# neeek2303/EMOPortraits

Measured on AMD Instinct MI355X. Metric: reenactment frames/sec @512x512, 1-src->N-driver, higher is better.
Workload: dtype f32

## Files before the change

### emoportraits_amd/csrc/conv_inst_f16x2_up2.hip

```cpp
#include "conv_dispatch.h"
#include "conv_igemm_bf16x3.h"
#include "conv_split_pair_common.h"

#ifndef EMO_UP2_CHAIN
#define EMO_UP2_CHAIN 1
#endif
#ifndef EMO_UP2_LOADS_EARLY
#define EMO_UP2_LOADS_EARLY 1
#endif

struct ConvCfgUp2 {
  static constexpr int BM = 64, TM = 2, TP = 2, KC = 16, NPL = 2;
  static constexpr int TRL = 2, TWL = 64;
  static constexpr int PR = TRL + 2, NQ = TWL / 4, NQ1 = NQ + 1;
  static constexpr int SUB = ((PR * NQ1 + 4 + 11) / 16) * 16 + 4;
  static constexpr int CHS = 4 * SUB, NG = 2, QPG = 128, NHQ = 2 * PR;
  static constexpr int WPLANE = 2 * BM;
  static constexpr int WTAP = NPL * WPLANE;
  static constexpr int WST = 8 * WTAP;
  static constexpr int WST_BYTES = WST * 16;
  static constexpr int PPL = NG * CHS, PBUF = NPL * PPL;
  static constexpr int SCT = 1024;
  static constexpr int OFF_P = 0, OFF_W = 2 * PBUF, OFF_SCT = OFF_W + WST;
  static constexpr int WSTRIDE = WST + (2 * SCT + BM) / 4;
  static constexpr int OFF_BIAS_F = OFF_SCT * 4 + 2 * SCT;
  static constexpr int EPI_CS = 4 * 132 + 4;
  static constexpr int OFF_IMG_F = (OFF_W + WSTRIDE) * 4;
  static constexpr int LDS_BYTES = (OFF_IMG_F + 32 * EPI_CS) * 4;
  static_assert(OFF_IMG_F >= OFF_BIAS_F + BM, "the epilogue image spares the patch buffers, W[0], the tables and the bias: a chained successor's");
  static_assert(32 * EPI_CS * 4 >= WST_BYTES, "W[1] lies inside the image's allocation");
  static_assert(WST_BYTES == 32 * 1024, "eight 1 KiB pieces per wave and half-stage");
  static_assert(PR * NQ + NHQ <= QPG, "one interior quad or one halo pixel per thread and stage");
  static_assert(LDS_BYTES <= 160 * 1024, "LDS");
};

__global__ __launch_bounds__(256) __attribute__((amdgpu_waves_per_eu(1, 1)))
void conv_igemm_f16x2_up2_kernel(const ConvArgs a) {
  using Cfg = ConvCfgUp2;
  using opx8 = halfx8;
  constexpr int NPL = 2, NPROD = 3;
  constexpr int BM = Cfg::BM, TM = Cfg::TM, TP = Cfg::TP, KC = Cfg::KC;
  constexpr int PR = Cfg::PR, NQ = Cfg::NQ, NQ1 = Cfg::NQ1, SUB = Cfg::SUB, CHS = Cfg::CHS, QPG = Cfg::QPG;
  constexpr int NHQ = Cfg::NHQ, PPL = Cfg::PPL, PBUF = Cfg::PBUF;
  constexpr bool UPS = false;
  constexpr int TW = Cfg::TWL, TWS = Cfg::TWL;

  extern __shared__ __attribute__((aligned(16))) float smem[];

  const int tid = threadIdx.x;
  const int lane = tid & 63;
  const int wave = __builtin_amdgcn_readfirstlane(tid >> 6);
  const int half = lane >> 5, l32 = lane & 31;
  const int wq = wave & 1;
  const int p0 = (wave >> 1) * TP * 32;
  float sat_m = 0.0f;

  const int HW = a.H * a.W;
  const bool has_affine = a.scale != nullptr;
  const float in_scale = a.in_scale;
  constexpr float CLAMP_HI = 65504.0f;
  const float clamp_lo = a.relu_in ? 0.0f : -CLAMP_HI;
  const int nst = a.n_cchunks;
  const int nptiles = a.tiles_x * a.tiles_y;

  const int q_u = tid % QPG;
  const int q_g = __builtin_amdgcn_readfirstlane(tid / QPG);
  const bool is_quad = q_u < PR * NQ;
  const int hq = q_u - PR * NQ;
  const bool is_halo = !is_quad && hq < NHQ;
  const int h_side = hq & 1;
  const int q_r = is_quad ? q_u / NQ : (is_halo ? hq >> 1 : 0);
  const int q_c = is_quad ? q_u - q_r * NQ : 0;
  int q_slb[4];
#pragma unroll
  for (int i = 0; i < 4; ++i) {
    const int dump = q_g * CHS + i * SUB + PR * NQ1 + (q_u & 3);
    const int own = is_quad ? q_g * CHS + i * SUB + q_r * NQ1 + q_c : q_g * CHS + h_side * SUB + q_r * NQ1 + NQ;
    q_slb[i] = ((is_quad || (is_halo && i == (h_side ? 0 : 3))) ? own : dump) * 16;
  }

  floatx16 acc_lo[2][TM][TP], acc_hi[2][TM][TP];

  const int q8 = a.n_work >> 3, r8 = a.n_work & 7;
  const int xcd = blockIdx.x & 7;
  const int n_mine = q8 + (xcd < r8 ? 1 : 0);
  const int l_base = xcd < r8 ? xcd * (q8 + 1) : r8 * (q8 + 1) + (xcd - r8) * q8;
  const int l_stride = (gridDim.x + 7) >> 3;
#define EMO_U_WPTR(c_, k_, p_) (reinterpret_cast<const char*>(a.wpk) + ((long)((c_) * nst + (k_)) * 2 + (p_)) * Cfg::WST_BYTES)

  const int a_off = (half * BM + l32) * 16;
  EMO_P_DECLARE_B_OFF()

  const char* const lds_c = reinterpret_cast<const char*>(smem);
  char* const lds_w = reinterpret_cast<char*>(smem);
  opx8 fa_[2][NPL][TM], fb_[2][NPL][TP];
#define EMO_U_LOAD_FRAGS_PLANE(set_, pl_, hb_, pbyte_, a_, b_)                                        \
  {                                                                                                   \
    _Pragma("unroll") for (int i = 0; i < TM; ++i)                                                    \
      fa_[set_][pl_][i] = *reinterpret_cast<const opx8*>(lds_c + a_off + (Cfg::OFF_W + (hb_) * Cfg::WSTRIDE + \
          ((wq * 4 + (a_) * 2 + (b_)) * NPL + (pl_)) * Cfg::WPLANE + i * 32) * 16);                   \
    _Pragma("unroll") for (int j = 0; j < TP; ++j)                                                    \
      fb_[set_][pl_][j] = *reinterpret_cast<const opx8*>(lds_c + (EMO_P_B_OFF(j, (hb_) + (a_), wq + (b_)) + (pbyte_)) + ((pl_) * PPL) * 16); \
  }

  float* const sct = smem + Cfg::OFF_SCT * 4;
  const unsigned smem_lds = (unsigned)(size_t)(__attribute__((address_space(3))) char*)reinterpret_cast<char*>(smem);
  const unsigned lane16 = (unsigned)lane * 16u;

  floatx4 qv[8];
  float q_lo, q_hi;
  int q_tix;
  floatx4 q_sc, q_sh;
  opx8 cv_h, cv_m;
  emo_intx4 xrs = emo_raw_buffer(a.x);
  unsigned usoff[8];
#pragma unroll
  for (int u = 0; u < 8; ++u) usoff[u] = (unsigned)__builtin_amdgcn_readfirstlane((int)((unsigned)u * (unsigned)HW * 4u));
  unsigned lq_off = 0;
  bool lq_ok = false;
  unsigned q_vo;
#define EMO_U_ISSUE_BEGIN(st_)                                                                        \
  {                                                                                                   \
    const int c0_ = (st_) * KC + q_g * 8;                                                             \
    const bool cv_ = c0_ < a.Cin;                                                                     \
    const int cs_ = cv_ ? c0_ : 0;                                                                    \
    const bool keep_ = lq_ok && cv_;                                                                  \
    q_lo = keep_ ? clamp_lo : 0.0f;                                                                   \
    q_hi = keep_ ? CLAMP_HI : 0.0f;                                                                   \
    q_vo = lq_off + (unsigned)cs_ * (unsigned)HW * 4u;                                                \
    q_tix = (has_affine ? cs_ : (cs_ & (Cfg::SCT - 1))) >> 2;                                         \
  }
#define EMO_U_ISSUE_LOADS(u0_, u1_)                                                                   \
  { _Pragma("unroll") for (int u = (u0_); u < (u1_); u += 2) emo_bload4x2_pinned(xrs, q_vo, usoff[u], usoff[u + 1], qv[u], qv[u + 1]); }
#define EMO_U_HALF_TABLE(hf_)                                                                         \
  {                                                                                                   \
    const floatx4* t4_ = reinterpret_cast<const floatx4*>(sct) + q_tix + (hf_);                       \
    q_sc = t4_[0]; q_sh = t4_[Cfg::SCT / 4];                                                          \
  }
#define EMO_U_TOUCH_QUAD() { _Pragma("unroll") for (int u = 0; u < 8; ++u) emo_touch4(qv[u]); }
#define EMO_U_CONV_PIXEL(pbyte_, i_)                                                                  \
  {                                                                                                   \
    _Pragma("unroll") for (int hf_ = 0; hf_ < 2; ++hf_) {                                             \
      EMO_U_HALF_TABLE(hf_)                                                                           \
      float t_[4];                                                                                    \
      _Pragma("unroll") for (int k = 0; k < 4; ++k)                                                   \
        t_[k] = __fmaf_rn(qv[4 * hf_ + k][i_], q_sc[k], q_sh[k]);                                     \
      sat_m = __builtin_fmaxf(__builtin_fmaxf(sat_m, __builtin_fabsf(t_[0])), __builtin_fabsf(t_[1])); \
      sat_m = __builtin_fmaxf(__builtin_fmaxf(sat_m, __builtin_fabsf(t_[2])), __builtin_fabsf(t_[3])); \
      _Pragma("unroll") for (int k = 0; k < 4; k += 2)                                                \
        emo_split_f16x2_pair(__builtin_amdgcn_fmed3f(t_[k], q_lo, q_hi), __builtin_amdgcn_fmed3f(t_[k + 1], q_lo, q_hi), \
                             cv_h, cv_m, 4 * hf_ + k);                                                \
    }                                                                                                 \
    char* d_ = lds_w + (q_slb[i_] + (pbyte_));                                                        \
    *reinterpret_cast<opx8*>(d_) = cv_h;                                                              \
    *reinterpret_cast<opx8*>(d_ + PPL * 16) = cv_m;                                                   \
  }
#define EMO_U_DMA_PIECE(ptr_, wb_, k_)                                                                \
  {                                                                                                   \
    const int j_ = wave + 4 * (k_);                                                                   \
    emo_dma16_pinned_s((ptr_) + j_ * 1024, lane16, smem_lds + (unsigned)((Cfg::OFF_W + (wb_) * Cfg::WSTRIDE) * 16 + j_ * 1024)); \
  }

  constexpr int PA3[3] = {1, 0, 0}, PB3[3] = {0, 1, 0};
  constexpr int NTE = Cfg::SCT / 256;

#define EMO_U_DECODE(P_, L_)                                                                          \
  {                                                                                                   \
    const int l_ = (L_);                                                                              \
    P_##cotile = __builtin_amdgcn_readfirstlane(l_ % a.n_cotiles);                                    \
    const int rest_ = l_ / a.n_cotiles;                                                               \
    P_##n = __builtin_amdgcn_readfirstlane(rest_ / nptiles);                                          \
    const int lt_ = rest_ - P_##n * nptiles;                                                          \
    P_##x0 = __builtin_amdgcn_readfirstlane((lt_ % a.tiles_x) * Cfg::TWL);        \
    P_##y0 = __builtin_amdgcn_readfirstlane((lt_ / a.tiles_x) * Cfg::TRL);                            \
  }
#define EMO_U_CURSOR_OF(P_, ok_, off_)                                                                \
  {                                                                                                   \
    const int q_y_ = P_##y0 - 1 + q_r;                                                                \
    const int q_x_ = is_quad ? P_##x0 + 4 * q_c : (h_side ? P_##x0 + TWS : P_##x0 - 4);               \
    ok_ = (is_quad || is_halo) && (unsigned)q_y_ < (unsigned)a.H && q_x_ >= 0 && q_x_ < a.W;          \
    off_ = ok_ ? (unsigned)(q_y_ * a.W + q_x_) * 4u : 0u;                                             \
  }
#define EMO_U_NEXT_STAGE_BEGIN()                                                                      \
  {                                                                                                   \
    const bool sw_ = chain_out && cg + 2 == nst;                                                      \
    const int tgt_ = (chain_out && cg + 2 >= nst) ? cg + 2 - nst : (cg + 2 < nst ? cg + 2 : nst - 1); \
    lq_ok = sw_ ? nxq_ok : lq_ok;                                                                     \
    lq_off = sw_ ? nxq_off : lq_off;                                                                  \
    EMO_U_ISSUE_BEGIN(tgt_)                                                                           \
  }
#if EMO_S_TIMING == 2
#define EMO_U_LOOP_BARRIER(n_)                                                                        \
  {                                                                                                   \
    const unsigned long long b0_ = __builtin_amdgcn_s_memtime();                                      \
    asm volatile("s_waitcnt vmcnt(%0) lgkmcnt(0)" ::"n"(n_) : "memory");                              \
    const unsigned long long b1_ = __builtin_amdgcn_s_memtime();                                      \
    asm volatile("s_waitcnt lgkmcnt(0)\n\ts_barrier" ::: "memory");                                  \
    const unsigned long long b2_ = __builtin_amdgcn_s_memtime();                                      \
    asm volatile("s_waitcnt lgkmcnt(0)" ::: "memory");                                                \
    tw_wait += b1_ - b0_; tw_bar += b2_ - b1_; ++tw_n;                                                \
  }
#else
#define EMO_U_LOOP_BARRIER(n_) EMO_P_BARRIER(n_)
#endif

  constexpr bool CHAIN = EMO_UP2_CHAIN != 0, LOADS_EARLY = EMO_UP2_LOADS_EARLY != 0;
  float te_b = 0.0f;
  bool chained_in = false;
  int pp = 0;
  for (int idx8 = blockIdx.x >> 3; idx8 < n_mine; idx8 += l_stride) {
#if EMO_S_TIMING
    unsigned long long tstamp[12];
    for (int k = 0; k < 12; ++k) tstamp[k] = 0;
    unsigned long long tw_wait = 0, tw_bar = 0, tw_n = 0;
#endif
    EMO_S_STAMP(0)
    int cotile, it_n, x0, y0;
    {
      int it_cotile, it_x0, it_y0;
      EMO_U_DECODE(it_, l_base + idx8)
      cotile = it_cotile; x0 = it_x0; y0 = it_y0;
    }
    int nx_cotile = 0, nx_n = 0, nx_x0 = 0, nx_y0 = 0;
    bool chain_out = false, nxq_ok = false;
    unsigned nxq_off = 0;
    if (CHAIN && idx8 + l_stride < n_mine) {
      EMO_U_DECODE(nx_, l_base + idx8 + l_stride)
      chain_out = nx_n == it_n && nst >= 2;
      EMO_U_CURSOR_OF(nx_, nxq_ok, nxq_off)
    }
    xrs = emo_raw_buffer(a.x + (long)it_n * a.Cin * HW);
    asm volatile("" : "=v"(cv_h));
    asm volatile("" : "=v"(cv_m));
    if (CHAIN && chained_in) {
      if (tid < BM) smem[Cfg::OFF_BIAS_F + tid] = te_b;
      const char* const w1_ = EMO_U_WPTR(cotile, 0, 1);
      EMO_U_DMA_PIECE(w1_, 1, 0)
      EMO_U_DMA_PIECE(w1_, 1, 1)
      EMO_P_BARRIER(40);
    } else {
      {
        int it_x0 = x0, it_y0 = y0;
        EMO_U_CURSOR_OF(it_, lq_ok, lq_off)
      }
#pragma unroll
      for (int u = 0; u < 8; ++u) asm volatile("" : "=v"(qv[u]));
      {
        const char* const w0_ = EMO_U_WPTR(cotile, 0, 0);
#pragma unroll
        for (int k = 0; k < 8; ++k) EMO_U_DMA_PIECE(w0_, 0, k)
        const char* const w1_ = EMO_U_WPTR(cotile, 0, 1);
        EMO_U_DMA_PIECE(w1_, 1, 0)
        EMO_U_DMA_PIECE(w1_, 1, 1)
      }
      EMO_U_ISSUE_BEGIN(0)
      EMO_U_ISSUE_LOADS(0, 8)
#pragma unroll
      for (int k = 0; k < NTE; ++k) {
        const int c = tid + 256 * k;
        if (c < min(a.Cin, Cfg::SCT)) {
          const bool real = has_affine;
          sct[c] = (real ? a.scale[(long)it_n * a.Cin + c] : 1.0f) * in_scale;
          sct[Cfg::SCT + c] = (real ? a.shift[(long)it_n * a.Cin + c] : 0.0f) * in_scale;
        }
      }
      if (tid < BM) smem[Cfg::OFF_BIAS_F + tid] = a.bias != nullptr ? a.bias[cotile * BM + tid] : 0.0f;
      EMO_P_WAIT(0);
      EMO_U_TOUCH_QUAD()
      __syncthreads();
#pragma unroll
      for (int i = 0; i < 4; ++i) EMO_U_CONV_PIXEL(Cfg::OFF_P * 16, i)
      EMO_U_ISSUE_BEGIN(nst > 1 ? 1 : 0)
      EMO_U_ISSUE_LOADS(0, 8)
      EMO_P_BARRIER(0);
      EMO_U_TOUCH_QUAD()
      pp = 0;
    }

    EMO_S_STAMP(1)
#pragma unroll
    for (int c = 0; c < 2; ++c)
#pragma unroll
      for (int i = 0; i < TM; ++i)
#pragma unroll
        for (int j = 0; j < TP; ++j)
#pragma unroll
          for (int r = 0; r < 16; ++r) { acc_lo[c][i][j][r] = 0.0f; acc_hi[c][i][j][r] = 0.0f; }
    {
      const int pb0_ = (Cfg::OFF_P + pp * PBUF) * 16;
#pragma unroll
      for (int pl = 0; pl < NPL; ++pl) EMO_U_LOAD_FRAGS_PLANE(0, pl, 0, pb0_, 0, 0)
    }
    for (int cg = 0; cg < nst; ++cg) {
      const int pcur_b = (Cfg::OFF_P + pp * PBUF) * 16, pnxt_b = (Cfg::OFF_P + (pp ^ 1) * PBUF) * 16;
      const bool last_ = cg + 1 >= nst;
#pragma unroll
      for (int h = 0; h < 2; ++h) {
        const bool past_ = last_ && chain_out;
        const bool have1_ = CHAIN || h == 0 || !last_, have2_ = !last_ || (CHAIN && h == 0);
        const int ce_ = past_ ? nx_cotile : cotile, ke_ = last_ ? (chain_out ? 0 : nst - 1) : cg + 1;
        const char* const dma1 = h == 0 ? EMO_U_WPTR(cotile, cg, 1) : EMO_U_WPTR(ce_, ke_, 0);
        const char* const dma2 = EMO_U_WPTR(ce_, ke_, h);
        if (EMO_CONV_SETPRIO) __builtin_amdgcn_s_setprio(1);
#pragma unroll
        for (int gs = 0; gs < 4; ++gs) {
          const int fcur = (h * 4 + gs) & 1, fnxt = fcur ^ 1;
          if (gs == 3) { EMO_U_LOOP_BARRIER(0); }
          if (gs == 3 && h == 1) EMO_U_TOUCH_QUAD()
          if (!LOADS_EARLY && gs == 0 && h == 1) EMO_U_NEXT_STAGE_BEGIN()
          __builtin_amdgcn_sched_barrier(0);
          {
            const int an = gs < 3 ? (gs + 1) >> 1 : 0, bn = gs < 3 ? (gs + 1) & 1 : 0;
            const int hbn = gs < 3 ? h : h ^ 1;
            const int pbn = (gs == 3 && h == 1) ? pnxt_b : pcur_b;
#pragma unroll
            for (int pl = 0; pl < NPL; ++pl) {
              EMO_U_LOAD_FRAGS_PLANE(fnxt, pl, hbn, pbn, an, bn)
              if (gs < 3 && have1_) EMO_U_DMA_PIECE(dma1, h ^ 1, 2 + 2 * gs + pl)
              if (gs == 3 && have2_) EMO_U_DMA_PIECE(dma2, h, pl)
              if (!LOADS_EARLY && h == 1 && gs == 0) EMO_U_ISSUE_LOADS(2 * pl, 2 * pl + 2)
              if (!LOADS_EARLY && h == 1 && gs > 0 && gs < 3 && pl == 0) EMO_U_ISSUE_LOADS(2 + 2 * gs, 4 + 2 * gs)
            }
          }
          if (h == 0) EMO_U_CONV_PIXEL(pnxt_b, gs)
          if (LOADS_EARLY && h == 0 && gs == 3) {
            EMO_U_NEXT_STAGE_BEGIN()
            EMO_U_ISSUE_LOADS(0, 8)
          }
#pragma unroll
          for (int p = 0; p < NPROD; ++p) {
            const int pa = PA3[p], pb = PB3[p];
#pragma unroll
            for (int i = 0; i < TM; ++i)
#pragma unroll
              for (int j = 0; j < TP; ++j) {
                floatx16& acc_ = (pa == 0 && pb == 0) ? acc_lo[h][i][j] : acc_hi[h][i][j];
                acc_ = __builtin_amdgcn_mfma_f32_32x32x16_f16(fb_[fcur][pb][j], fa_[fcur][pa][i], acc_, 0, 0, 0);
              }
          }
          __builtin_amdgcn_sched_barrier(0);
        }
        if (EMO_CONV_SETPRIO) __builtin_amdgcn_s_setprio(0);
      }
      pp ^= 1;
    }

    EMO_S_STAMP(2)
    EMO_P_WAIT(0);
    EMO_S_STAMP(5)
    __syncthreads();
    EMO_S_STAMP(6)
    EMO_S_STAMP(7)
    float* const img = smem + Cfg::OFF_IMG_F;
    if (CHAIN && chain_out && tid < BM) te_b = a.bias != nullptr ? a.bias[nx_cotile * BM + tid] : 0.0f;
    const bool want_stats = a.gn_stats != nullptr;
    const int Ho = a.Hl, Wo = a.Wl;
    const unsigned oplane = (unsigned)Ho * Wo;
    const int tiles_xo = Wo / 64;
    const int ec = tid >> 4, eu = tid & 15;
#pragma unroll
    for (int i = 0; i < TM; ++i) {
#pragma unroll
      for (int p = 0; p < 2; ++p)
#pragma unroll
        for (int j = 0; j < TP; ++j)
#pragma unroll
          for (int r = 0; r < 16; ++r) {
            const float v = (emo_acc_read(acc_lo[p][i][j][r]) + emo_acc_read(acc_hi[p][i][j][r])) * a.out_scale;
            const int m = (r >> 2) * 8 + half * 4 + (r & 3);
            const int hr = 2 * (wave >> 1) + p, col = 2 * (j * 32 + m) + wq;
            img[l32 * Cfg::EPI_CS + hr * 132 + col] = v;
          }
      __syncthreads();
#pragma unroll
      for (int cc = 0; cc < 2; ++cc) {
        const int c = cc * 16 + ec;
        const int co = cotile * BM + i * 32 + c;
        const float bs = smem[Cfg::OFF_BIAS_F + i * 32 + c];
        float* const obase = a.out + ((long)it_n * a.Cout + co) * oplane;
        float s_[2] = {0.0f, 0.0f};
        floatx4 v_[4][2];
#pragma unroll
        for (int hr = 0; hr < 4; ++hr)
#pragma unroll
          for (int k = 0; k < 2; ++k) {
            floatx4 v = *reinterpret_cast<const floatx4*>(img + c * Cfg::EPI_CS + hr * 132 + 4 * eu + 64 * k);
            v = v + floatx4{bs, bs, bs, bs};
            v_[hr][k] = v;
            float* const op = obase + (unsigned)(2 * y0 + hr) * Wo + (2 * x0 + 4 * eu + 64 * k);
            if (EMO_CONV_NT_STORE) __builtin_nontemporal_store(v, reinterpret_cast<floatx4*>(op));
            else *reinterpret_cast<floatx4*>(op) = v;
            s_[k] += (v[0] + v[1]) + (v[2] + v[3]);
          }
        if (want_stats) {
          emo_row16_sum_n<2>(s_);
          float m2_[2] = {0.0f, 0.0f};
#pragma unroll
          for (int k = 0; k < 2; ++k) {
            s_[k] *= 1.0f / 256.0f;
#pragma unroll
            for (int hr = 0; hr < 4; ++hr)
#pragma unroll
              for (int e = 0; e < 4; ++e) {
                const float d = v_[hr][k][e] - s_[k];
                m2_[k] = __fmaf_rn(d, d, m2_[k]);
              }
          }
          emo_row16_sum_n<2>(m2_);
          if (eu == 0) {
#pragma unroll
            for (int k = 0; k < 2; ++k) {
              const int ptile = (y0 >> 1) * tiles_xo + (x0 >> 5) + k;
              reinterpret_cast<float2*>(a.gn_stats)[((long)it_n * (oplane / 256) + ptile) * a.Cout + co] = make_float2(s_[k], m2_[k]);
            }
          }
        }
      }
      if (i == 0) {
        EMO_S_STAMP(8)
        __syncthreads();
      }
    }
    EMO_S_STAMP(9)
#if EMO_S_TIMING
    EMO_S_STAMP(3)
    asm volatile("s_waitcnt vmcnt(0)" ::: "memory");
    EMO_S_STAMP(4)
    {
      const int ep_L_ = l_base + idx8;
      if (tid == 0 && ep_L_ < EMO_S_TLOG_N) {
        unsigned long long* t_ = emo_s_tlog + (long)ep_L_ * EMO_S_TLOG_W;
#pragma unroll
        for (int k = 0; k < 12; ++k) t_[k] = tstamp[k];
        t_[12] = (unsigned long long)__builtin_amdgcn_s_getreg((31 << 11) | 4);
        t_[13] = (unsigned long long)__builtin_amdgcn_s_getreg((31 << 11) | 20);
        t_[14] = (unsigned long long)blockIdx.x;
        t_[15] = (unsigned long long)(chained_in ? 1 : 0);
      }
      if (EMO_S_TIMING == 2 && lane == 0 && ep_L_ < EMO_S_TLOG_N / 8) {
        unsigned long long* w_ = emo_s_tlog + ((long)EMO_S_TLOG_N / 4 + (long)ep_L_ * 4 + wave) * EMO_S_TLOG_W;
        w_[0] = tw_wait; w_[1] = tw_bar; w_[2] = tw_n; w_[3] = tstamp[2] - tstamp[1];
      }
    }
#endif
    __syncthreads();
    chained_in = chain_out;
  }
  if (a.sat_flag != nullptr && sat_m > 65504.0f) *a.sat_flag = 1;
#undef EMO_U_WPTR
#undef EMO_U_DECODE
#undef EMO_U_CURSOR_OF
#undef EMO_U_NEXT_STAGE_BEGIN
#undef EMO_U_LOOP_BARRIER
#undef EMO_U_LOAD_FRAGS_PLANE
#undef EMO_U_ISSUE_BEGIN
#undef EMO_U_ISSUE_LOADS
#undef EMO_U_HALF_TABLE
#undef EMO_U_TOUCH_QUAD
#undef EMO_U_CONV_PIXEL
#undef EMO_U_DMA_PIECE
}

int conv_f16x2_up2_launch(ConvArgs a, hipStream_t s) {
  using Cfg = ConvCfgUp2;
  if (a.KD != 1 || a.D != 1 || a.ksplit != 1 || a.res != nullptr || a.act != EMO_ACT_NONE || a.run_if != nullptr) return EMO_ERR_UNSUPPORTED;
  if (a.Cout % Cfg::BM || a.Cin % 8 || (a.scale && a.Cin > Cfg::SCT)) return EMO_ERR_UNSUPPORTED;
  if (a.W % Cfg::TWL || a.H % Cfg::TRL) return EMO_ERR_UNSUPPORTED;
  if ((reinterpret_cast<unsigned long long>(a.x) & 15ull) || (reinterpret_cast<unsigned long long>(a.out) & 15ull)) return EMO_ERR_ALIGN;
  if ((unsigned long long)a.Cin * a.H * a.W * 4ull >= (1ull << 32) || (long)a.Hl * a.Wl >= (1l << 31)) return EMO_ERR_UNSUPPORTED;
  const long nt = (long)(a.W / Cfg::TWL) * (a.H / Cfg::TRL);
  const int cot = a.Cout / Cfg::BM;
  if (a.N > 65535 || nt * cot * a.N > 0x7fffffffL) return EMO_ERR_UNSUPPORTED;
  auto kern = conv_igemm_f16x2_up2_kernel;
  const int rc = emo_raise_dynamic_lds(kern);
  if (rc != EMO_OK) return rc;
  a.tiles_x = a.W / Cfg::TWL;
  a.tiles_y = a.H / Cfg::TRL;
  a.tiles_z = 1;
  a.n_cchunks = (a.Cin + Cfg::KC - 1) / Cfg::KC;
  a.stages_per_split = a.n_cchunks;
  a.partial = nullptr;
  a.cot0 = 0;
  a.n_cotiles = cot;
  a.n_work = (int)(nt * cot * a.N);
  const int ncu = emo_cu_count();
  const int grid = a.n_work > ncu ? ncu : a.n_work;
  hipLaunchKernelGGL(kern, dim3((unsigned)grid), dim3(256), (size_t)Cfg::LDS_BYTES, s, a);
  return emo_launch_status();
}

#if EMO_S_TIMING
extern "C" int emo_debug_conv_timing_up2(unsigned long long* host_out, int n_items) {
  if (!host_out || n_items < 0 || n_items > EMO_S_TLOG_N) return EMO_ERR_BAD_ARG;
  if (hipDeviceSynchronize() != hipSuccess) return EMO_ERR_BAD_ARG;
  return hipMemcpyFromSymbol(host_out, HIP_SYMBOL(emo_s_tlog), (size_t)n_items * EMO_S_TLOG_W * sizeof(unsigned long long)) == hipSuccess ? EMO_OK : EMO_ERR_BAD_ARG;
}
#endif
```

Before: 401.0.

## Double up2 conv tile height and merge split accumulators into one set

Raises the low-res tile from 2 to 4 rows (TP 2→4) so each weight stage feeds twice as many pixels, cutting weight DMA per output. It drops the lo/hi split accumulators so register use stays bounded, and chains the MFMAs into a single accumulator. The epilogue becomes a row-pair-by-row-pair pass with a smaller LDS image and more barriers, and it adds a partial-tile guard for heights not divisible by 4. Risks are a longer serial MFMA dependency chain, more epilogue syncs and fewer work items for load balance.

Result: faster. 413.1, median of 6 (+3.0%).

```diff
diff --git a/emoportraits_amd/csrc/conv_inst_f16x2_up2.hip b/emoportraits_amd/csrc/conv_inst_f16x2_up2.hip
--- a/emoportraits_amd/csrc/conv_inst_f16x2_up2.hip
+++ b/emoportraits_amd/csrc/conv_inst_f16x2_up2.hip
@@ -10,8 +10,8 @@
 #endif
 
 struct ConvCfgUp2 {
-  static constexpr int BM = 64, TM = 2, TP = 2, KC = 16, NPL = 2;
-  static constexpr int TRL = 2, TWL = 64;
+  static constexpr int BM = 64, TM = 2, TP = 4, KC = 16, NPL = 2;
+  static constexpr int TRL = 4, TWL = 64;
   static constexpr int PR = TRL + 2, NQ = TWL / 4, NQ1 = NQ + 1;
   static constexpr int SUB = ((PR * NQ1 + 4 + 11) / 16) * 16 + 4;
   static constexpr int CHS = 4 * SUB, NG = 2, QPG = 128, NHQ = 2 * PR;
@@ -24,11 +24,13 @@
   static constexpr int OFF_P = 0, OFF_W = 2 * PBUF, OFF_SCT = OFF_W + WST;
   static constexpr int WSTRIDE = WST + (2 * SCT + BM) / 4;
   static constexpr int OFF_BIAS_F = OFF_SCT * 4 + 2 * SCT;
-  static constexpr int EPI_CS = 4 * 132 + 4;
+  static constexpr int EPI_CS = 4 * 64 + 4;
+  static constexpr int EPI_CH = 32;
   static constexpr int OFF_IMG_F = (OFF_W + WSTRIDE) * 4;
-  static constexpr int LDS_BYTES = (OFF_IMG_F + 32 * EPI_CS) * 4;
+  static constexpr int LDS_BYTES = (OFF_IMG_F + EPI_CH * EPI_CS) * 4;
   static_assert(OFF_IMG_F >= OFF_BIAS_F + BM, "the epilogue image spares the patch buffers, W[0], the tables and the bias: a chained successor's");
-  static_assert(32 * EPI_CS * 4 >= WST_BYTES, "W[1] lies inside the image's allocation");
+  static_assert(EPI_CH * EPI_CS * 4 >= WST_BYTES, "W[1] lies inside the image's allocation");
+  static_assert(TRL == 4 && TP == 4, "a wave holds two low-res rows: one epilogue pass is one row pair's 4 high-res rows");
   static_assert(WST_BYTES == 32 * 1024, "eight 1 KiB pieces per wave and half-stage");
   static_assert(PR * NQ + NHQ <= QPG, "one interior quad or one halo pixel per thread and stage");
   static_assert(LDS_BYTES <= 160 * 1024, "LDS");
@@ -79,7 +81,7 @@
     q_slb[i] = ((is_quad || (is_halo && i == (h_side ? 0 : 3))) ? own : dump) * 16;
   }
 
-  floatx16 acc_lo[2][TM][TP], acc_hi[2][TM][TP];
+  floatx16 acc[2][TM][TP];
 
   const int q8 = a.n_work >> 3, r8 = a.n_work & 7;
   const int xcd = blockIdx.x & 7;
@@ -237,7 +239,7 @@
       const char* const w1_ = EMO_U_WPTR(cotile, 0, 1);
       EMO_U_DMA_PIECE(w1_, 1, 0)
       EMO_U_DMA_PIECE(w1_, 1, 1)
-      EMO_P_BARRIER(40);
+      EMO_P_BARRIER(63);
     } else {
       {
         int it_x0 = x0, it_y0 = y0;
@@ -285,7 +287,7 @@
 #pragma unroll
         for (int j = 0; j < TP; ++j)
 #pragma unroll
-          for (int r = 0; r < 16; ++r) { acc_lo[c][i][j][r] = 0.0f; acc_hi[c][i][j][r] = 0.0f; }
+          for (int r = 0; r < 16; ++r) acc[c][i][j][r] = 0.0f;
     {
       const int pb0_ = (Cfg::OFF_P + pp * PBUF) * 16;
 #pragma unroll
@@ -333,10 +335,8 @@
 #pragma unroll
             for (int i = 0; i < TM; ++i)
 #pragma unroll
-              for (int j = 0; j < TP; ++j) {
-                floatx16& acc_ = (pa == 0 && pb == 0) ? acc_lo[h][i][j] : acc_hi[h][i][j];
-                acc_ = __builtin_amdgcn_mfma_f32_32x32x16_f16(fb_[fcur][pb][j], fa_[fcur][pa][i], acc_, 0, 0, 0);
-              }
+              for (int j = 0; j < TP; ++j)
+                acc[h][i][j] = __builtin_amdgcn_mfma_f32_32x32x16_f16(fb_[fcur][pb][j], fa_[fcur][pa][i], acc[h][i][j], 0, 0, 0);
           }
           __builtin_amdgcn_sched_barrier(0);
         }
@@ -361,65 +361,72 @@
 #pragma unroll
     for (int i = 0; i < TM; ++i) {
 #pragma unroll
-      for (int p = 0; p < 2; ++p)
-#pragma unroll
-        for (int j = 0; j < TP; ++j)
-#pragma unroll
-          for (int r = 0; r < 16; ++r) {
-            const float v = (emo_acc_read(acc_lo[p][i][j][r]) + emo_acc_read(acc_hi[p][i][j][r])) * a.out_scale;
-            const int m = (r >> 2) * 8 + half * 4 + (r & 3);
-            const int hr = 2 * (wave >> 1) + p, col = 2 * (j * 32 + m) + wq;
-            img[l32 * Cfg::EPI_CS + hr * 132 + col] = v;
-          }
-      __syncthreads();
-#pragma unroll
-      for (int cc = 0; cc < 2; ++cc) {
-        const int c = cc * 16 + ec;
-        const int co = cotile * BM + i * 32 + c;
-        const float bs = smem[Cfg::OFF_BIAS_F + i * 32 + c];
-        float* const obase = a.out + ((long)it_n * a.Cout + co) * oplane;
-        float s_[2] = {0.0f, 0.0f};
-        floatx4 v_[4][2];
-#pragma unroll
-        for (int hr = 0; hr < 4; ++hr)
+      for (int g = 0; g < 2; ++g) {
+        if (y0 + 2 * g < a.H) {
 #pragma unroll
           for (int k = 0; k < 2; ++k) {
-            floatx4 v = *reinterpret_cast<const floatx4*>(img + c * Cfg::EPI_CS + hr * 132 + 4 * eu + 64 * k);
-            v = v + floatx4{bs, bs, bs, bs};
-            v_[hr][k] = v;
-            float* const op = obase + (unsigned)(2 * y0 + hr) * Wo + (2 * x0 + 4 * eu + 64 * k);
-            if (EMO_CONV_NT_STORE) __builtin_nontemporal_store(v, reinterpret_cast<floatx4*>(op));
-            else *reinterpret_cast<floatx4*>(op) = v;
-            s_[k] += (v[0] + v[1]) + (v[2] + v[3]);
-          }
-        if (want_stats) {
-          emo_row16_sum_n<2>(s_);
-          float m2_[2] = {0.0f, 0.0f};
-#pragma unroll
-          for (int k = 0; k < 2; ++k) {
-            s_[k] *= 1.0f / 256.0f;
-#pragma unroll
-            for (int hr = 0; hr < 4; ++hr)
-#pragma unroll
-              for (int e = 0; e < 4; ++e) {
-                const float d = v_[hr][k][e] - s_[k];
-                m2_[k] = __fmaf_rn(d, d, m2_[k]);
+            if (i + g + k > 0) __syncthreads();
+            if ((wave >> 1) == g) {
+#pragma unroll
+              for (int p = 0; p < 2; ++p)
+#pragma unroll
+                for (int jj = 0; jj < 2; ++jj)
+#pragma unroll
+                  for (int r4 = 0; r4 < 4; ++r4) {
+                    floatx4 v;
+#pragma unroll
+                    for (int e = 0; e < 4; ++e) v[e] = emo_acc_read(acc[p][i][2 * jj + k][4 * r4 + e]) * a.out_scale;
+                    const int m = r4 * 8 + half * 4;
+                    *reinterpret_cast<floatx4*>(img + l32 * Cfg::EPI_CS + (2 * jj + p) * 64 + wq * 32 + m) = v;
+                  }
+            }
+            __syncthreads();
+            const int ptile = ((y0 >> 1) + g) * tiles_xo + (x0 >> 5) + k;
+            float s_[2] = {0.0f, 0.0f};
+            floatx4 v_[2][4];
+#pragma unroll
+            for (int cc = 0; cc < 2; ++cc) {
+              const int c = cc * 16 + ec;
+              const float bs = smem[Cfg::OFF_BIAS_F + i * 32 + c];
+              float* const obase = a.out + ((long)it_n * a.Cout + cotile * BM + i * 32 + c) * oplane;
+#pragma unroll
+              for (int hr = 0; hr < 4; ++hr) {
+                const float2 e0 = *reinterpret_cast<const float2*>(img + c * Cfg::EPI_CS + hr * 64 + 2 * eu);
+                const float2 e1 = *reinterpret_cast<const float2*>(img + c * Cfg::EPI_CS + hr * 64 + 32 + 2 * eu);
+                const floatx4 v = floatx4{e0.x, e1.x, e0.y, e1.y} + floatx4{bs, bs, bs, bs};
+                v_[cc][hr] = v;
+                float* const op = obase + (unsigned)(2 * y0 + 4 * g + hr) * Wo + (2 * x0 + 64 * k + 4 * eu);
+                if (EMO_CONV_NT_STORE) __builtin_nontemporal_store(v, reinterpret_cast<floatx4*>(op));
+                else *reinterpret_cast<floatx4*>(op) = v;
+                s_[cc] += (v[0] + v[1]) + (v[2] + v[3]);
               }
-          }
-          emo_row16_sum_n<2>(m2_);
-          if (eu == 0) {
-#pragma unroll
-            for (int k = 0; k < 2; ++k) {
-              const int ptile = (y0 >> 1) * tiles_xo + (x0 >> 5) + k;
-              reinterpret_cast<float2*>(a.gn_stats)[((long)it_n * (oplane / 256) + ptile) * a.Cout + co] = make_float2(s_[k], m2_[k]);
+            }
+            if (want_stats) {
+              emo_row16_sum_n<2>(s_);
+              float m2_[2] = {0.0f, 0.0f};
+#pragma unroll
+              for (int cc = 0; cc < 2; ++cc) {
+                s_[cc] *= 1.0f / 256.0f;
+#pragma unroll
+                for (int hr = 0; hr < 4; ++hr)
+#pragma unroll
+                  for (int e = 0; e < 4; ++e) {
+                    const float d = v_[cc][hr][e] - s_[cc];
+                    m2_[cc] = __fmaf_rn(d, d, m2_[cc]);
+                  }
+              }
+              emo_row16_sum_n<2>(m2_);
+              if (eu == 0) {
+#pragma unroll
+                for (int cc = 0; cc < 2; ++cc)
+                  reinterpret_cast<float2*>(a.gn_stats)[((long)it_n * (oplane / 256) + ptile) * a.Cout + cotile * BM + i * 32 + cc * 16 + ec] =
+                      make_float2(s_[cc], m2_[cc]);
+              }
             }
           }
         }
       }
-      if (i == 0) {
-        EMO_S_STAMP(8)
-        __syncthreads();
-      }
+      if (i == 0) { EMO_S_STAMP(8) }
     }
     EMO_S_STAMP(9)
 #if EMO_S_TIMING
@@ -465,17 +472,17 @@
   using Cfg = ConvCfgUp2;
   if (a.KD != 1 || a.D != 1 || a.ksplit != 1 || a.res != nullptr || a.act != EMO_ACT_NONE || a.run_if != nullptr) return EMO_ERR_UNSUPPORTED;
   if (a.Cout % Cfg::BM || a.Cin % 8 || (a.scale && a.Cin > Cfg::SCT)) return EMO_ERR_UNSUPPORTED;
-  if (a.W % Cfg::TWL || a.H % Cfg::TRL) return EMO_ERR_UNSUPPORTED;
+  if (a.W % Cfg::TWL || a.H % 2) return EMO_ERR_UNSUPPORTED;
   if ((reinterpret_cast<unsigned long long>(a.x) & 15ull) || (reinterpret_cast<unsigned long long>(a.out) & 15ull)) return EMO_ERR_ALIGN;
   if ((unsigned long long)a.Cin * a.H * a.W * 4ull >= (1ull << 32) || (long)a.Hl * a.Wl >= (1l << 31)) return EMO_ERR_UNSUPPORTED;
-  const long nt = (long)(a.W / Cfg::TWL) * (a.H / Cfg::TRL);
+  const long nt = (long)(a.W / Cfg::TWL) * ((a.H + Cfg::TRL - 1) / Cfg::TRL);
   const int cot = a.Cout / Cfg::BM;
   if (a.N > 65535 || nt * cot * a.N > 0x7fffffffL) return EMO_ERR_UNSUPPORTED;
   auto kern = conv_igemm_f16x2_up2_kernel;
   const int rc = emo_raise_dynamic_lds(kern);
   if (rc != EMO_OK) return rc;
   a.tiles_x = a.W / Cfg::TWL;
-  a.tiles_y = a.H / Cfg::TRL;
+  a.tiles_y = (a.H + Cfg::TRL - 1) / Cfg::TRL;
   a.tiles_z = 1;
   a.n_cchunks = (a.Cin + Cfg::KC - 1) / Cfg::KC;
   a.stages_per_split = a.n_cchunks;
```
